# LasseWolter/laughter-detection-icsi

Measured on AMD Instinct MI355X. Metric: 1 s@16 kHz segments/sec (featurize+ResNet fwd/bwd), higher is better.
Workload: dtype f32 (64->64 and 32->32 convolutions: f16x2 split operands with per-tile power-of-two scales, f32 accumulate; error vs float64 within 1.5x of the exact-f32 kernels'); 1 GPU; BASELINE configs[2]: end-to-end featurize (HIP fbank 44 mel) + ResNetBigger resnet_base fwd/bwd + clip + Adam, random labels, dropout 0.5; global_batch=512, parallelism=dp1, overlap_wgrad=False, overlap_wgrad_small=True, bf16x3_convs=True, f16x2_convs=True, relu_bits=True, virtual_a1=True

## Files before the change

laughter-detection-icsi_amd/csrc/conv_h2.hip:

```cpp
#include "lad_common.h"
#include "lad_device.h"
#include "lad_b3_tile.h"
#include "lad_bn_math.h"
#include "lad_h2.h"

#include <algorithm>
#include <cstdlib>

namespace {
using namespace lad;
using namespace lad::b3t;

constexpr int KC = 32;
constexpr int ROWB = 128;
constexpr int FPIECES = KC * 4 / 16;

template <int C>
struct H2 {
    static constexpr int NSTAGE = C / KC;
    static constexpr int NCT = C / 16;
    static constexpr int PLANE_B = NCT * 1024;
    static constexpr int TAP_BYTES = 2 * PLANE_B;
    static constexpr int IMG_BYTES = TAPS * NSTAGE * TAP_BYTES;
    static constexpr int TAIL_BYTES = 16;
};

struct PackRec {
    const float *w;
    unsigned char *wt;
    int mode;
    int channels;
};
constexpr int PACK_SPLIT = 16;
template <int C>
__device__ __forceinline__ void pack_h2_image(const PackRec &rec, int part) {
    using K = H2<C>;
    __shared__ float smax[K::NSTAGE][16];
    __shared__ int kexp[K::NSTAGE];
    const int tid = threadIdx.x, lane = tid & 63, wave = tid >> 6;
    float m[K::NSTAGE];
#pragma unroll
    for (int s = 0; s < K::NSTAGE; ++s) m[s] = 0.f;
    static_assert((C * TAPS) % 4 == 0, "float4 groups stay inside one (co, ci range)");
    for (int idx4 = tid; idx4 < C * C * TAPS / 4; idx4 += 1024) {
        const float4 v = reinterpret_cast<const float4 *>(rec.w)[idx4];
        const float a[4] = {fabsf(v.x), fabsf(v.y), fabsf(v.z), fabsf(v.w)};
#pragma unroll
        for (int j = 0; j < 4; ++j) {
            const int idx = idx4 * 4 + j;
            const int co = idx / (C * TAPS), ci = (idx / TAPS) % C;
            const int k = rec.mode == 0 ? ci : co;
#pragma unroll
            for (int s = 0; s < K::NSTAGE; ++s) m[s] = (k / KC == s) ? fmaxf(m[s], a[j]) : m[s];
        }
    }
#pragma unroll
    for (int s = 0; s < K::NSTAGE; ++s) {
        const float v = wave_max64_dpp(m[s]);
        if (lane == 0) smax[s][wave] = v;
    }
    __syncthreads();
    if (tid < K::NSTAGE) {
        float v = 0.f;
        for (int w = 0; w < 16; ++w) v = fmaxf(v, smax[tid][w]);
        kexp[tid] = scale_exp(v);
        if (part == 0) reinterpret_cast<int *>(rec.wt + K::IMG_BYTES)[tid] = kexp[tid];
    }
    __syncthreads();
    unsigned short *out = reinterpret_cast<unsigned short *>(rec.wt);
    constexpr int SHARE = K::IMG_BYTES / 2 / PACK_SPLIT;
    for (int idx = part * SHARE + tid; idx < (part + 1) * SHARE; idx += 1024) {
        int t = idx;
        const int e = t & 7; t >>= 3;
        const int n = t & 15; t >>= 4;
        const int kq = t & 3; t >>= 2;
        const int ct = t % K::NCT; t /= K::NCT;
        const int plane = t & 1; t >>= 1;
        const int stage = t % K::NSTAGE;
        const int tap = t / K::NSTAGE;
        const int k = stage * KC + kq * 8 + e;
        const int nn = ct * 16 + n;
        const int co = rec.mode == 0 ? nn : k, ci = rec.mode == 0 ? k : nn;
        const int src_tap = rec.mode == 0 ? tap : TAPS - 1 - tap;
        const float v = rec.w[((int64_t)co * C + ci) * TAPS + src_tap] * pow2f(kexp[stage]);
        const _Float16 h1 = (_Float16)v;
        const _Float16 h2 = (_Float16)(v - (float)h1);
        out[idx] = __builtin_bit_cast(unsigned short, plane == 0 ? h1 : h2);
    }
}
template <int C>
__global__ __launch_bounds__(1024) void pack_h2_kernel(const PackRec *__restrict__ recs) {
    const PackRec rec = recs[blockIdx.x / PACK_SPLIT];
    const int part = blockIdx.x % PACK_SPLIT;
    if (C == 64 || (C == 0 && rec.channels == 64)) pack_h2_image<64>(rec, part);
    else pack_h2_image<32>(rec, part);
}

#ifdef LAD_STAMP
__device__ unsigned long long lad_dbg_h2[16 * 16384];
#define LAD_H2_STAMP(k) \
    if (threadIdx.x == 0 && blockIdx.x < 16384) lad_dbg_h2[blockIdx.x * 16 + (k)] = __builtin_amdgcn_s_memtime();
#else
#define LAD_H2_STAMP(k)
#endif

constexpr int NSLOT = 3;
constexpr int H2_EPI_ANY = -1;
constexpr int h2_epi(bool bias, int addend, bool partials, bool from_bits) {
    return (bias ? 1 : 0) | (addend << 1) | (partials ? 8 : 0) | (from_bits ? 16 : 0);
}
template <int C, int RB, bool STAT, bool INBN, int EPI>
__global__ __launch_bounds__(THREADS, RB == 1 ? 3 : 2) void conv_h2_kernel(const float *__restrict__ in, const unsigned char *__restrict__ wt,
                                                             const float *__restrict__ bias, const float *addend,
                                                             const unsigned long long *__restrict__ abits, float *out,
                                                             float *__restrict__ partials, Geom g, B3Stat bst,
                                                             const float *__restrict__ in_coef) {
    using K = H2<C>;
    constexpr int NSTAGE = K::NSTAGE, NCT = K::NCT, PLANE_B = K::PLANE_B, TAP_BYTES = K::TAP_BYTES;
    constexpr int TMW = TM * RB, NRT = 2 * RB;
    constexpr int NPRE = ((TMW + 2 * 47) * FPIECES + THREADS - 1) / THREADS;
    constexpr int CPS = TAPS;
    constexpr int KP = (CPS - NSLOT) < CPS / 2 ? (CPS - NSLOT) : CPS / 2;
    static_assert(CPS % NSLOT == 0 && NPRE <= 32, "every stage starts in ring slot 0; staging geometry");
    extern __shared__ __attribute__((aligned(128))) unsigned char smem_b[];
    const int tid = threadIdx.x, lane = tid & 63, wave = __builtin_amdgcn_readfirstlane(tid >> 6);
    const int halo = g.Wp + 1;
    const int nrows = TMW + 2 * halo;
    const int main_bytes = max(NSLOT * TAP_BYTES + nrows * ROWB, TM * (C + 4) * 4);
    unsigned char *b_s = smem_b;
    unsigned char *a_s = b_s + NSLOT * TAP_BYTES;
    unsigned char *mask_s = smem_b + main_bytes;
    float *smax = reinterpret_cast<float *>(mask_s + TMW);
    const unsigned per_x = (gridDim.x + 7u) / 8u;
    const unsigned tile_id = (blockIdx.x % 8u) * per_x + blockIdx.x / 8u;
    const int64_t q0 = (int64_t)tile_id * TMW;
    if (q0 >= g.rows) return;

    LAD_H2_STAMP(0)
    constexpr int NW_TAP = TAP_BYTES / (THREADS * 16);
    static_assert(TAP_BYTES % (THREADS * 16) == 0 && NW_TAP >= 1, "the DMA count per tap must not depend on the wave");
    auto issue_tap = [&](int tap, int stage, int slot) {
        const unsigned char *src = wt + (int64_t)(tap * NSTAGE + stage) * TAP_BYTES;
        unsigned char *dst = b_s + slot * TAP_BYTES;
#pragma unroll
        for (int r = 0; r < NW_TAP; ++r)
            dma16(src + (r * THREADS + tid) * 16, lds_addr(dst + (r * THREADS + wave * 64) * 16));
    };
    const int *wexp = reinterpret_cast<const int *>(wt + K::IMG_BYTES);

    const int64_t start = q0 - halo;
    const int64_t first = start < 0 ? 0 : start;
    const int row_lo = (int)(first - start);
    const int64_t span_rows = min(g.rows - first, (int64_t)(nrows - row_lo));
    auto voff = [&](int u) {
        const int idx = u * THREADS + tid;
        return idx < nrows * FPIECES ? ((idx >> 3) - row_lo) * (C * 4) + (idx & 7) * 16 : -1;
    };
    auto stage_rsrc = [&](int stage) {
        return make_rsrc(reinterpret_cast<const unsigned char *>(in) + first * (C * 4) + stage * (KC * 4), span_rows * (C * 4) - stage * (KC * 4));
    };
    unsigned keep_bits = 0;
    u32x4 pre[NPRE];
    auto activate = [&](int stage) {
        float m = 0.f;
        f32x4 sc = {0.f, 0.f, 0.f, 0.f}, sh = sc;
        if (INBN) {
            sc = *reinterpret_cast<const f32x4 *>(in_coef + stage * KC + (tid & 7) * 4);
            sh = *reinterpret_cast<const f32x4 *>(in_coef + C + stage * KC + (tid & 7) * 4);
        }
#pragma unroll
        for (int u = 0; u < NPRE; ++u) {
            if (INBN) pre[u] = bn_relu_piece(pre[u], sc, sh, (keep_bits >> u) & 1u);
            const float4 f = as_f4(pre[u]);
            m = fmaxf(fmaxf(m, fmaxf(fabsf(f.x), fabsf(f.y))), fmaxf(fabsf(f.z), fabsf(f.w)));
        }
        m = wave_max64_dpp(m);
        if (lane == 0) smax[wave] = m;
    };
    auto tile_exp = [&]() { return scale_exp(fmaxf(fmaxf(smax[0], smax[1]), fmaxf(smax[2], smax[3]))); };
    auto put_all = [&](float scl) {
#pragma unroll
        for (int u = 0; u < NPRE; ++u) {
            const int idx = u * THREADS + tid;
            if (idx < nrows * FPIECES) {
                const int row = idx >> 3, piece = idx & 7;
                const float4 f = as_f4(pre[u]);
                unsigned a1, a2, b1, b2;
                split2_pair(f.x * scl, f.y * scl, a1, a2);
                split2_pair(f.z * scl, f.w * scl, b1, b2);
                const unsigned off = (unsigned)row * ROWB + ((((piece >> 1) ^ (row & 6)) << 4) | ((piece & 1) << 3));
                *reinterpret_cast<u32x2 *>(a_s + off) = u32x2{a1, b1};
                *reinterpret_cast<u32x2 *>(a_s + (off ^ 64u)) = u32x2{a2, b2};
            }
        }
    };

    {
        const __amdgpu_buffer_rsrc_t in_r = stage_rsrc(0);
#pragma unroll
        for (int u = 0; u < NPRE; ++u) pre[u] = buf_load16(in_r, voff(u));
    }
#pragma unroll
    for (int k = 0; k < NSLOT - 1; ++k) issue_tap(k, 0, k);
    for (int j = tid; j < TMW; j += THREADS) mask_s[j] = interior_row32((uint32_t)q0 + (uint32_t)j, g) ? 1 : 0;
    if (INBN) {
#pragma unroll
        for (int u = 0; u < NPRE; ++u)
            keep_bits |= (interior_row32((uint32_t)(start + ((u * THREADS + tid) >> 3)), g) ? 1u : 0u) << u;
    }
    LAD_H2_STAMP(1)
    activate(0);
    __syncthreads();
    int ktot = tile_exp() + wexp[0];
    put_all(pow2f(ktot - wexp[0]));
    LAD_H2_STAMP(2)

    const int m = lane & 15, kq = lane >> 4;
    const int rl = wave * 32 + m + halo - 1;
    const unsigned char *b_lane = b_s + kq * 256 + m * 16;

    f32x4 acc[NRT][NCT];
#pragma unroll
    for (int r = 0; r < NRT; ++r)
#pragma unroll
        for (int c = 0; c < NCT; ++c) acc[r][c] = f32x4{0.f, 0.f, 0.f, 0.f};

#pragma unroll
    for (int stage = 0; stage < NSTAGE; ++stage) {
        const bool last = stage + 1 == NSTAGE;
#pragma unroll
        for (int tap = 0; tap < TAPS; ++tap) {
            const int kc = tap;
            const int slot = kc % NSLOT;
            {
                constexpr int YOUNGER = NSLOT - 2;
                if (!last) {
                    if (kc > KP && kc <= KP + NSLOT - 1) wait_dma_fixed<YOUNGER, NPRE, NW_TAP>();
                    else wait_dma_fixed<YOUNGER, 0, NW_TAP>();
                } else {
                    if (CPS - 1 - kc >= YOUNGER) wait_dma_fixed<YOUNGER, 0, NW_TAP>();
                    else wait_dma_fixed<0, 0, NW_TAP>();
                }
                __syncthreads();
                const int kn = kc + NSLOT - 1;
                if (kn < CPS) issue_tap(kn, stage, kn % NSLOT);
                else if (!last) issue_tap(kn - CPS, stage + 1, kn % NSLOT);
                if (kc == KP && !last) {
                    const __amdgpu_buffer_rsrc_t in_r = stage_rsrc(stage + 1);
#pragma unroll
                    for (int u = 0; u < NPRE; ++u) pre[u] = buf_load16(in_r, voff(u));
                }
            }
            const int rt = rl + (tap / 3 - 1) * g.Wp + (tap % 3);
            const unsigned a1o = (unsigned)rt * ROWB + ((unsigned)(kq ^ (rt & 6)) << 4);
            const unsigned a2o = a1o ^ 64u;
            const int boff = slot * TAP_BYTES;
            f16x8 a1[NRT], a2[NRT];
#pragma unroll
            for (int r = 0; r < NRT; ++r) {
                const int roff = ((r >> 1) * TM + (r & 1) * 16) * ROWB;
                a1[r] = *reinterpret_cast<const f16x8 *>(a_s + a1o + roff);
                a2[r] = *reinterpret_cast<const f16x8 *>(a_s + a2o + roff);
            }
#pragma unroll
            for (int c = 0; c < NCT; ++c) {
                const f16x8 b1 = *reinterpret_cast<const f16x8 *>(b_lane + boff + c * 1024);
                const f16x8 b2 = *reinterpret_cast<const f16x8 *>(b_lane + boff + PLANE_B + c * 1024);
#pragma unroll
                for (int r = 0; r < NRT; ++r) acc[r][c] = __builtin_amdgcn_mfma_f32_16x16x32_f16(a1[r], b2, acc[r][c], 0, 0, 0);
#pragma unroll
                for (int r = 0; r < NRT; ++r) acc[r][c] = __builtin_amdgcn_mfma_f32_16x16x32_f16(a2[r], b1, acc[r][c], 0, 0, 0);
#pragma unroll
                for (int r = 0; r < NRT; ++r) acc[r][c] = __builtin_amdgcn_mfma_f32_16x16x32_f16(a1[r], b1, acc[r][c], 0, 0, 0);
            }
        }
#ifdef LAD_STAMP
        if (threadIdx.x == 0 && blockIdx.x < 16384) lad_dbg_h2[blockIdx.x * 16 + 3 + 2 * stage] = __builtin_amdgcn_s_memtime();
#endif
        if (!last) {
            activate(stage + 1);
            __syncthreads();
            const int kw = wexp[stage + 1];
            const int kn = min(tile_exp() + kw, ktot + 8);
            const int d = kn - ktot;
            if (d != 0) {
#pragma unroll
                for (int r = 0; r < NRT; ++r)
#pragma unroll
                    for (int c = 0; c < NCT; ++c)
#pragma unroll
                        for (int j = 0; j < 4; ++j) acc[r][c][j] = __builtin_ldexpf(acc[r][c][j], d);
            }
            ktot = kn;
            const int ka = kn - kw;
            put_all(ka >= -126 ? pow2f(ka) : 0.f);
        }
#ifdef LAD_STAMP
        if (threadIdx.x == 0 && blockIdx.x < 16384) lad_dbg_h2[blockIdx.x * 16 + 4 + 2 * stage] = __builtin_amdgcn_s_memtime();
#endif
    }
    __syncthreads();
    LAD_H2_STAMP(11)
#pragma unroll
    for (int rb = 0; rb < RB; ++rb) {
        const int64_t qs = q0 + rb * TM;
        if (rb > 0) {
            if (qs >= g.rows) break;
            __syncthreads();
        }
        auto store_acc = [&](float *my) {
#pragma unroll
            for (int rr = 0; rr < 2; ++rr)
#pragma unroll
                for (int c = 0; c < NCT; ++c)
#pragma unroll
                    for (int j = 0; j < 4; ++j)
                        my[(rr * 16 + (lane >> 4) * 4 + j) * (C + 4) + c * 16 + m] = __builtin_ldexpf(acc[rb * 2 + rr][c][j], -ktot);
        };
        if constexpr (EPI == H2_EPI_ANY)
            b3_epilogue<C, STAT>(store_acc, bias, addend, abits, out, partials, mask_s + rb * TM, reinterpret_cast<float *>(smem_b), qs, g.rows, bst);
        else
            h2_epilogue<C, STAT, (EPI & 1) != 0, (EPI >> 1) & 3, (EPI & 8) != 0, (EPI & 16) != 0>(
                store_acc, bias, addend, abits, out, partials, mask_s + rb * TM, reinterpret_cast<float *>(smem_b), qs, g.rows, bst);
    }
    LAD_H2_STAMP(12)
}

template <int C, int RB>
size_t h2_lds_bytes(const Geom &g) {
    using K = H2<C>;
    const int nrows = TM * RB + 2 * (g.Wp + 1);
    const size_t main_bytes = std::max<size_t>(NSLOT * K::TAP_BYTES + (size_t)nrows * ROWB, (size_t)TM * (C + 4) * 4);
    return main_bytes + TM * RB + 16;
}

int h2_two_rounds() {
    static int n = 0;
    if (n == 0) {
        int dev = 0;
        hipDeviceProp_t prop;
        n = (hipGetDevice(&dev) == hipSuccess && hipGetDeviceProperties(&prop, dev) == hipSuccess && prop.multiProcessorCount > 0)
                ? 4 * prop.multiProcessorCount : 1024;
    }
    return n;
}

struct H2Args {
    const float *in, *in_coef;
    const unsigned char *wt;
    const float *bias, *addend;
    const unsigned long long *abits;
    float *out, *partials;
    B3Stat bst;
    Geom g;
    hipStream_t stream;
};

template <int C, int RB, bool STAT, bool INBN, int EPI>
int launch_h2_form(const H2Args &a) {
    static lad::DeviceOnce attr_set;
    if (!attr_set) {
        LAD_HIP_CHECK(hipFuncSetAttribute((const void *)conv_h2_kernel<C, RB, STAT, INBN, EPI>, hipFuncAttributeMaxDynamicSharedMemorySize, 96 * 1024));
        attr_set = true;
    }
    const int64_t tiles = ceil_div(a.g.rows, TM * RB);
    hipLaunchKernelGGL((conv_h2_kernel<C, RB, STAT, INBN, EPI>), dim3((unsigned)(ceil_div(tiles, 8) * 8)), dim3(THREADS), (h2_lds_bytes<C, RB>(a.g)),
                       a.stream, a.in, a.wt, a.bias, a.addend, a.abits, a.out, a.partials, a.g, a.bst, a.in_coef);
    return check_launch("conv_h2_kernel");
}

template <int C, int RB, bool STAT, bool INBN>
int launch_h2_rb(const H2Args &a) {
    const int form = h2_epi(a.bias != nullptr, a.addend == nullptr ? H2_ADD_NONE : a.abits == nullptr ? H2_ADD_PLAIN : H2_ADD_GATED,
                            a.partials != nullptr, STAT && a.bst.bits != nullptr);
#define LAD_H2_FORM(...)                                                                                                           \
    if (form == h2_epi(__VA_ARGS__)) return launch_h2_form<C, RB, STAT, INBN, h2_epi(__VA_ARGS__)>(a);
    if constexpr (STAT) {
        LAD_H2_FORM(false, H2_ADD_NONE, true, false)
        LAD_H2_FORM(false, H2_ADD_GATED, true, true)
    } else {
        LAD_H2_FORM(true, H2_ADD_NONE, true, false)
        LAD_H2_FORM(true, H2_ADD_PLAIN, true, false)
        if constexpr (!INBN) {
            LAD_H2_FORM(false, H2_ADD_NONE, false, false)
            LAD_H2_FORM(false, H2_ADD_PLAIN, false, false)
            LAD_H2_FORM(false, H2_ADD_GATED, false, false)
        }
    }
#undef LAD_H2_FORM
    return launch_h2_form<C, RB, STAT, INBN, H2_EPI_ANY>(a);
}

template <int C, bool STAT, bool INBN>
int launch_h2(const float *in, const float *in_coef, const void *wt, const float *bias, const float *addend, const uint64_t *abits,
              float *out, float *partials, const B3Stat &bst, int64_t batch, int32_t H, int32_t W, void *stream, const char *who) {
    const Geom g = make_geom(batch, H, W);
    LAD_REQUIRE(g.rows < ((int64_t)1 << 31) && g.img < (1 << 20), "%s: more than 2^31 rows, or an image of more than 2^20 positions", who);
    LAD_REQUIRE(W <= 46, "%s: image too wide for the tile (W = %d)", who, W);
    const H2Args a{in, in_coef, (const unsigned char *)wt, bias, addend, (const unsigned long long *)abits, out, partials, bst, g, (hipStream_t)stream};
    if (ceil_div(g.rows, TM * 2) < h2_two_rounds()) return launch_h2_rb<C, 1, STAT, INBN>(a);
    return launch_h2_rb<C, 2, STAT, INBN>(a);
}
}

extern "C" int64_t lad_conv_h2_packed_weight_bytes(int32_t channels) {
    if (channels == 64) return H2<64>::IMG_BYTES + H2<64>::TAIL_BYTES;
    if (channels == 32) return H2<32>::IMG_BYTES + H2<32>::TAIL_BYTES;
    return -1;
}

extern "C" int lad_conv_h2_pack_weights_multi(const void *table, int32_t n, int32_t channels, void *stream) {
    using namespace lad;
    LAD_REQUIRE(table && n >= 1, "lad_conv_h2_pack_weights_multi: empty table");
    static_assert(sizeof(PackRec) == 24, "record layout");
    if (channels == 64) hipLaunchKernelGGL(pack_h2_kernel<64>, dim3(n * PACK_SPLIT), dim3(1024), 0, (hipStream_t)stream, (const PackRec *)table);
    else if (channels == 32) hipLaunchKernelGGL(pack_h2_kernel<32>, dim3(n * PACK_SPLIT), dim3(1024), 0, (hipStream_t)stream, (const PackRec *)table);
    else if (channels == 0) hipLaunchKernelGGL(pack_h2_kernel<0>, dim3(n * PACK_SPLIT), dim3(1024), 0, (hipStream_t)stream, (const PackRec *)table);
    else return fail(LAD_ERR_INVALID, "lad_conv_h2_pack_weights_multi: 64 or 32 channels, or 0 = per record (got %d)", channels);
    return check_launch("pack_h2_kernel");
}

extern "C" int lad_conv_h2(const float *in, const float *in_coef, const void *wt, const float *bias, const float *addend,
                           const uint64_t *addend_bits, float *out, float *partials, const float *bn_x, const uint64_t *bn_bits,
                           const float *bn_coef, int64_t batch, int32_t H, int32_t W, int32_t channels, void *stream) {
    using namespace lad;
    const char *who = "lad_conv_h2";
    LAD_REQUIRE(batch >= 1 && H >= 1 && W >= 1, "%s: bad geometry", who);
    LAD_REQUIRE(in && wt && out, "%s: null buffer", who);
    LAD_REQUIRE(addend_bits == nullptr || addend != nullptr, "%s: sign bits without an addend", who);
    LAD_REQUIRE((const void *)in != (const void *)out, "%s: the convolution cannot run in place", who);
    const bool stat = bn_x != nullptr;
    LAD_REQUIRE(!stat || (partials && bn_coef), "%s: the BatchNorm sums need partials and bn_coef", who);
    LAD_REQUIRE(stat || bn_bits == nullptr, "%s: bn_bits without bn_x", who);
    LAD_REQUIRE(!(stat && in_coef), "%s: an input BatchNorm and the backward sums are not combined", who);
    LAD_REQUIRE(channels == 64 || (addend_bits == nullptr && bn_bits == nullptr), "%s: sign bits are kept for 64-channel activations only", who);
    const B3Stat bst{bn_x, (const unsigned long long *)bn_bits, bn_coef};
    if (channels == 64) {
        if (stat) return launch_h2<64, true, false>(in, nullptr, wt, bias, addend, addend_bits, out, partials, bst, batch, H, W, stream, who);
        if (in_coef) return launch_h2<64, false, true>(in, in_coef, wt, bias, addend, addend_bits, out, partials, bst, batch, H, W, stream, who);
        return launch_h2<64, false, false>(in, nullptr, wt, bias, addend, addend_bits, out, partials, bst, batch, H, W, stream, who);
    }
    if (channels == 32) {
        if (stat) return launch_h2<32, true, false>(in, nullptr, wt, bias, addend, addend_bits, out, partials, bst, batch, H, W, stream, who);
        if (in_coef) return launch_h2<32, false, true>(in, in_coef, wt, bias, addend, addend_bits, out, partials, bst, batch, H, W, stream, who);
        return launch_h2<32, false, false>(in, nullptr, wt, bias, addend, addend_bits, out, partials, bst, batch, H, W, stream, who);
    }
    return fail(LAD_ERR_INVALID, "%s: 64 or 32 channels (got %d)", who, channels);
}

#ifdef LAD_STAMP
extern "C" int lad_debug_read_h2_stamps(unsigned long long *host_dst, int64_t n) {
    return hipMemcpyFromSymbol(host_dst, HIP_SYMBOL(lad_dbg_h2), n * sizeof(unsigned long long)) == hipSuccess ? 0 : -2;
}
#endif
```

laughter-detection-icsi_amd/csrc/lad_b3_tile.h:

```cpp
#pragma once
#include "lad_common.h"
#include "lad_device.h"

namespace lad {
namespace b3t {

constexpr int TAPS = 9;
constexpr int TM = 128;
constexpr int THREADS = 256;

struct B3Stat {
    const float *x;
    const unsigned long long *bits;
    const float *coef;
};

struct B3Scatter {
    const int *rowoff;
    int64_t base_row;
    int64_t span_rows;
    int64_t part_tile;
};

template <int C, bool STAT, bool SCATTER = false, class StoreAcc, class MaskT>
__device__ __forceinline__ void b3_epilogue(StoreAcc store_acc, const float *__restrict__ bias, const float *addend,
                                            const unsigned long long *__restrict__ abits, float *out, float *__restrict__ partials,
                                            const MaskT *mask_tile, float *out_s, int64_t q0, int64_t rows, const B3Stat &bst,
                                            const B3Scatter &sct = B3Scatter{nullptr, 0, 0, 0}) {
    constexpr int LDO = C + 4, LPR = C / 4, RPI = 64 / LPR, ITER = 32 / RPI, STEP = RPI * C * 4;
    const int tid = (int)threadIdx.x, lane = tid & 63, wave = tid >> 6;
    float *my = out_s + wave * 32 * LDO;
    store_acc(my);
    const int c4 = lane % LPR, rsub = lane / LPR;
    const int64_t row0 = SCATTER ? sct.base_row : q0;
    const int64_t tile_rows = SCATTER ? sct.span_rows : rows - q0;
    const int64_t tile_bytes = tile_rows * (C * 4);
    const int voff = ((wave * 32 + rsub) * C + c4 * 4) * 4;
    const int woff = (wave * 32 + rsub) * 8;
    int ro[SCATTER ? ITER : 1];
    if (SCATTER) {
#pragma unroll
        for (int it = 0; it < ITER; ++it) ro[it] = sct.rowoff[wave * 32 + it * RPI + rsub];
    }
    auto off16 = [&](int it) { return SCATTER ? (ro[SCATTER ? it : 0] < 0 ? -1 : ro[SCATTER ? it : 0] * (C * 4) + c4 * 16) : voff + it * STEP; };
    auto off8 = [&](int it) { return SCATTER ? (ro[SCATTER ? it : 0] < 0 ? -1 : ro[SCATTER ? it : 0] * 8) : woff + it * RPI * 8; };
    const __amdgpu_buffer_rsrc_t out_r = make_rsrc(out + row0 * C, tile_bytes);
    f32x4 bv = {0.f, 0.f, 0.f, 0.f};
    if (bias != nullptr) bv = *reinterpret_cast<const f32x4 *>(bias + c4 * 4);
    f32x4 s1 = {0.f, 0.f, 0.f, 0.f}, s2 = s1;
    f32x4 fsc = s1, fsh = s1, mu = s1, is = s1, mul = s1, isl = s1;
    if (STAT) {
        fsc = *reinterpret_cast<const f32x4 *>(bst.coef + 0 * C + c4 * 4);
        fsh = *reinterpret_cast<const f32x4 *>(bst.coef + 1 * C + c4 * 4);
        mu = *reinterpret_cast<const f32x4 *>(bst.coef + 2 * C + c4 * 4);
        is = *reinterpret_cast<const f32x4 *>(bst.coef + 3 * C + c4 * 4);
        mul = *reinterpret_cast<const f32x4 *>(bst.coef + 4 * C + c4 * 4);
        isl = *reinterpret_cast<const f32x4 *>(bst.coef + 5 * C + c4 * 4);
    }
    const bool from_bits = STAT && bst.bits != nullptr;
    auto gate = [&](u32x4 v, u32x2 w) {
        const unsigned lo = w.x >> c4, hi = w.y >> c4;
        v.x = (lo & 1u) ? v.x : 0u;
        v.y = (lo & 0x10000u) ? v.y : 0u;
        v.z = (hi & 1u) ? v.z : 0u;
        v.w = (hi & 0x10000u) ? v.w : 0u;
        return v;
    };
    constexpr int NI = STAT ? ITER / 2 : ITER;
#pragma unroll
    for (int i0 = 0; i0 < ITER; i0 += NI) {
        u32x4 adv[NI], bx[STAT ? NI : 1];
        u32x2 wv[NI], bw[STAT ? NI : 1];
        if (addend != nullptr) {
            const __amdgpu_buffer_rsrc_t add_r = make_rsrc(addend + row0 * C, tile_bytes);
#pragma unroll
            for (int u = 0; u < NI; ++u) adv[u] = buf_load16(add_r, off16(i0 + u));
            if (abits != nullptr) {
                const __amdgpu_buffer_rsrc_t bits_r = make_rsrc(abits + row0, tile_rows * 8);
#pragma unroll
                for (int u = 0; u < NI; ++u) wv[u] = buf_load8(bits_r, off8(i0 + u));
            }
        }
        if (STAT) {
            const __amdgpu_buffer_rsrc_t x_r = make_rsrc(bst.x + row0 * C, tile_bytes);
#pragma unroll
            for (int u = 0; u < NI; ++u) bx[u] = buf_load16(x_r, off16(i0 + u));
            if (from_bits) {
                const __amdgpu_buffer_rsrc_t w_r = make_rsrc(bst.bits + row0, tile_rows * 8);
#pragma unroll
                for (int u = 0; u < NI; ++u) bw[u] = buf_load8(w_r, off8(i0 + u));
            }
        }
#pragma unroll
        for (int u = 0; u < NI; ++u) {
            const int it = i0 + u;
            const int row = it * RPI + rsub;
            const float keep = SCATTER ? (ro[SCATTER ? it : 0] < 0 ? 0.f : 1.f) : (float)mask_tile[wave * 32 + row];
            f32x4 t = *reinterpret_cast<const f32x4 *>(my + row * LDO + c4 * 4);
            t += bv;
            if (addend != nullptr) t += __builtin_bit_cast(f32x4, abits != nullptr ? gate(adv[u], wv[u]) : adv[u]);
            t *= keep;
            buf_store16(__builtin_bit_cast(u32x4, t), out_r, off16(it));
            if (!STAT) {
                s1 += t;
                s2 = __builtin_elementwise_fma(t, t, s2);
            } else {
                const f32x4 xv = __builtin_bit_cast(f32x4, bx[u]);
                f32x4 d;
                if (from_bits) {
                    d = __builtin_bit_cast(f32x4, gate(__builtin_bit_cast(u32x4, t), bw[u]));
                } else {
                    const f32x4 yv = __builtin_elementwise_fma(xv, fsc, fsh);
                    d.x = yv.x > 0.f ? t.x : 0.f;
                    d.y = yv.y > 0.f ? t.y : 0.f;
                    d.z = yv.z > 0.f ? t.z : 0.f;
                    d.w = yv.w > 0.f ? t.w : 0.f;
                }
                const f32x4 tx = (xv - mu) - mul;
                const f32x4 xh = __builtin_elementwise_fma(tx, is, tx * isl);
                s1 += d;
                s2 = __builtin_elementwise_fma(d, xh, s2);
            }
        }
    }
    if (partials == nullptr) return;
    *reinterpret_cast<f32x4 *>(my + (rsub * 2 + 0) * C + c4 * 4) = s1;
    *reinterpret_cast<f32x4 *>(my + (rsub * 2 + 1) * C + c4 * 4) = s2;
    __syncthreads();
    if (tid < 2 * C) {
        const int k = tid / C, co = tid - k * C;
        float s = 0.0f;
#pragma unroll
        for (int w = 0; w < 4; ++w)
#pragma unroll
            for (int rs = 0; rs < RPI; ++rs) s += out_s[w * 32 * LDO + (rs * 2 + k) * C + co];
        partials[((SCATTER ? sct.part_tile : q0 / TM) * 2 + k) * C + co] = s;
    }
}

enum : int { H2_ADD_NONE = 0, H2_ADD_PLAIN = 1, H2_ADD_GATED = 2 };
template <int C, bool STAT, bool HAS_BIAS, int ADDEND, bool HAS_PARTIALS, bool FROM_BITS, class StoreAcc>
__device__ __forceinline__ void h2_epilogue(StoreAcc store_acc, const float *__restrict__ bias, const float *addend,
                                            const unsigned long long *__restrict__ abits, float *out, float *__restrict__ partials,
                                            const unsigned char *mask_tile, float *out_s, int64_t q0, int64_t rows, const B3Stat &bst) {
    static_assert(!FROM_BITS || STAT, "sign bits of the consuming BatchNorm: STAT launches only");
    static_assert(!STAT || HAS_PARTIALS, "the BatchNorm sums need partials");
    constexpr int LDO = C + 4, LPR = C / 4, RPI = 64 / LPR, ITER = 32 / RPI, STEP = RPI * C * 4;
    const int tid = (int)threadIdx.x, lane = tid & 63, wave = tid >> 6;
    float *my = out_s + wave * 32 * LDO;
    store_acc(my);
    const int c4 = lane % LPR, rsub = lane / LPR;
    const int64_t tile_rows = rows - q0;
    const int64_t tile_bytes = tile_rows * (C * 4);
    const int voff = ((wave * 32 + rsub) * C + c4 * 4) * 4;
    const int woff = (wave * 32 + rsub) * 8;
    const __amdgpu_buffer_rsrc_t out_r = make_rsrc(out + q0 * C, tile_bytes);
    f32x4 bv = {0.f, 0.f, 0.f, 0.f};
    if constexpr (HAS_BIAS) bv = *reinterpret_cast<const f32x4 *>(bias + c4 * 4);
    f32x4 s1 = {0.f, 0.f, 0.f, 0.f}, s2 = s1;
    f32x4 fsc = s1, fsh = s1, mu = s1, is = s1, mul = s1, isl = s1;
    if constexpr (STAT) {
        if constexpr (!FROM_BITS) {
            fsc = *reinterpret_cast<const f32x4 *>(bst.coef + 0 * C + c4 * 4);
            fsh = *reinterpret_cast<const f32x4 *>(bst.coef + 1 * C + c4 * 4);
        }
        mu = *reinterpret_cast<const f32x4 *>(bst.coef + 2 * C + c4 * 4);
        is = *reinterpret_cast<const f32x4 *>(bst.coef + 3 * C + c4 * 4);
        mul = *reinterpret_cast<const f32x4 *>(bst.coef + 4 * C + c4 * 4);
        isl = *reinterpret_cast<const f32x4 *>(bst.coef + 5 * C + c4 * 4);
    }
    auto gate = [&](u32x4 v, u32x2 w) {
        const unsigned lo = w.x >> c4, hi = w.y >> c4;
        v.x = (lo & 1u) ? v.x : 0u;
        v.y = (lo & 0x10000u) ? v.y : 0u;
        v.z = (hi & 1u) ? v.z : 0u;
        v.w = (hi & 0x10000u) ? v.w : 0u;
        return v;
    };
    constexpr int NI = (STAT || ADDEND == H2_ADD_GATED) ? ITER / 2 : ITER;
#pragma unroll
    for (int i0 = 0; i0 < ITER; i0 += NI) {
        u32x4 adv[ADDEND != H2_ADD_NONE ? NI : 1], bx[STAT ? NI : 1];
        u32x2 wv[ADDEND == H2_ADD_GATED ? NI : 1], bw[FROM_BITS ? NI : 1];
        if constexpr (ADDEND != H2_ADD_NONE) {
            const __amdgpu_buffer_rsrc_t add_r = make_rsrc(addend + q0 * C, tile_bytes);
#pragma unroll
            for (int u = 0; u < NI; ++u) adv[u] = buf_load16(add_r, voff + (i0 + u) * STEP);
            if constexpr (ADDEND == H2_ADD_GATED) {
                const __amdgpu_buffer_rsrc_t bits_r = make_rsrc(abits + q0, tile_rows * 8);
#pragma unroll
                for (int u = 0; u < NI; ++u) wv[u] = buf_load8(bits_r, woff + (i0 + u) * RPI * 8);
            }
        }
        if constexpr (STAT) {
            const __amdgpu_buffer_rsrc_t x_r = make_rsrc(bst.x + q0 * C, tile_bytes);
#pragma unroll
            for (int u = 0; u < NI; ++u) bx[u] = buf_load16(x_r, voff + (i0 + u) * STEP);
            if constexpr (FROM_BITS) {
                const __amdgpu_buffer_rsrc_t w_r = make_rsrc(bst.bits + q0, tile_rows * 8);
#pragma unroll
                for (int u = 0; u < NI; ++u) bw[u] = buf_load8(w_r, woff + (i0 + u) * RPI * 8);
            }
        }
#pragma unroll
        for (int u = 0; u < NI; ++u) {
            const int it = i0 + u;
            const int row = it * RPI + rsub;
            const float keep = (float)mask_tile[wave * 32 + row];
            f32x4 t = *reinterpret_cast<const f32x4 *>(my + row * LDO + c4 * 4);
            t += bv;
            if constexpr (ADDEND == H2_ADD_GATED) t += __builtin_bit_cast(f32x4, gate(adv[u], wv[u]));
            else if constexpr (ADDEND == H2_ADD_PLAIN) t += __builtin_bit_cast(f32x4, adv[u]);
            t *= keep;
            buf_store16(__builtin_bit_cast(u32x4, t), out_r, voff + it * STEP);
            if constexpr (!STAT) {
                if constexpr (HAS_PARTIALS) {
                    s1 += t;
                    s2 = __builtin_elementwise_fma(t, t, s2);
                }
            } else {
                const f32x4 xv = __builtin_bit_cast(f32x4, bx[u]);
                f32x4 d;
                if constexpr (FROM_BITS) {
                    d = __builtin_bit_cast(f32x4, gate(__builtin_bit_cast(u32x4, t), bw[u]));
                } else {
                    const f32x4 yv = __builtin_elementwise_fma(xv, fsc, fsh);
                    d.x = yv.x > 0.f ? t.x : 0.f;
                    d.y = yv.y > 0.f ? t.y : 0.f;
                    d.z = yv.z > 0.f ? t.z : 0.f;
                    d.w = yv.w > 0.f ? t.w : 0.f;
                }
                const f32x4 tx = (xv - mu) - mul;
                const f32x4 xh = __builtin_elementwise_fma(tx, is, tx * isl);
                s1 += d;
                s2 = __builtin_elementwise_fma(d, xh, s2);
            }
        }
    }
    if constexpr (HAS_PARTIALS) {
        *reinterpret_cast<f32x4 *>(my + (rsub * 2 + 0) * C + c4 * 4) = s1;
        *reinterpret_cast<f32x4 *>(my + (rsub * 2 + 1) * C + c4 * 4) = s2;
        __syncthreads();
        if (tid < 2 * C) {
            const int k = tid / C, co = tid - k * C;
            float s = 0.0f;
#pragma unroll
            for (int w = 0; w < 4; ++w)
#pragma unroll
                for (int rs = 0; rs < RPI; ++rs) s += out_s[w * 32 * LDO + (rs * 2 + k) * C + co];
            partials[(q0 / TM * 2 + k) * C + co] = s;
        }
    }
}

template <int TAP_BYTES>
__device__ __forceinline__ int dma_per_tap(int wave) {
    int n = 0;
#pragma unroll
    for (int r = 0; r * THREADS * 16 < TAP_BYTES; ++r) n += ((r * THREADS + wave * 64) * 16 < TAP_BYTES) ? 1 : 0;
    return n;
}

template <int TAPS_YOUNGER, int EXTRA>
__device__ __forceinline__ void wait_dma(int nw_tap) {
    static_assert(2 * TAPS_YOUNGER + EXTRA <= 63, "vmcnt is a 6-bit field");
    if (nw_tap == 2) asm volatile("s_waitcnt vmcnt(%0)" ::"n"(2 * TAPS_YOUNGER + EXTRA) : "memory");
    else if (nw_tap == 1) asm volatile("s_waitcnt vmcnt(%0)" ::"n"(TAPS_YOUNGER + EXTRA) : "memory");
    else asm volatile("s_waitcnt vmcnt(%0)" ::"n"(EXTRA) : "memory");
}
template <int TAPS_YOUNGER, int EXTRA, int NW_TAP>
__device__ __forceinline__ void wait_dma_fixed() {
    static_assert(NW_TAP * TAPS_YOUNGER + EXTRA <= 63, "vmcnt is a 6-bit field");
    asm volatile("s_waitcnt vmcnt(%0)" ::"n"(NW_TAP * TAPS_YOUNGER + EXTRA) : "memory");
}

}
}
```

Baseline: 50110 segments/s.

## Prefetch epilogue addend/stat loads during last conv stage and pipeline sub-tiles

For RB==2 launches whose epilogue reads global data (addend, gate bits, BN input), the coefficient and first sub-tile loads are now issued during the last stage's final taps. This hides their latency behind the remaining MFMA work. The epilogue is restructured so each sub-tile issues the next sub-tile's loads (or the next row block's) before consuming the current ones, which double-buffers global reads. It also sets NI per config, and a sched_barrier fence is used for the widest case. In exchange it holds more registers live across the main loop, which risks spills or lower occupancy, and it adjusts the waitcnt accounting accordingly.

```diff
diff --git a/laughter-detection-icsi_amd/csrc/conv_h2.hip b/laughter-detection-icsi_amd/csrc/conv_h2.hip
--- a/laughter-detection-icsi_amd/csrc/conv_h2.hip
+++ b/laughter-detection-icsi_amd/csrc/conv_h2.hip
@@ -109,6 +109,18 @@
 constexpr int h2_epi(bool bias, int addend, bool partials, bool from_bits) {
     return (bias ? 1 : 0) | (addend << 1) | (partials ? 8 : 0) | (from_bits ? 16 : 0);
 }
+template <int C, int RB, bool STAT, int EPI>
+struct H2EpiPlan {
+    static constexpr int ADDEND = EPI == H2_EPI_ANY ? H2_ADD_NONE : (EPI >> 1) & 3;
+    static constexpr bool FROM_BITS = EPI != H2_EPI_ANY && (EPI & 16) != 0;
+    static constexpr bool READS = EPI != H2_EPI_ANY && (STAT || ADDEND != H2_ADD_NONE);
+    static constexpr bool AHEAD = READS && RB == 2;
+    static constexpr int ITER = 32 / (64 / (C / 4));
+    static constexpr bool WIDEST = FROM_BITS && ADDEND == H2_ADD_GATED;
+    static constexpr int NI = (STAT || ADDEND == H2_ADD_GATED) && (RB == 1 || WIDEST) ? ITER / 2 : ITER;
+    static constexpr int TAP = TAPS - NSLOT;
+    static constexpr bool FENCE = AHEAD && WIDEST;
+};
 template <int C, int RB, bool STAT, bool INBN, int EPI>
 __global__ __launch_bounds__(THREADS, RB == 1 ? 3 : 2) void conv_h2_kernel(const float *__restrict__ in, const unsigned char *__restrict__ wt,
                                                              const float *__restrict__ bias, const float *addend,
@@ -225,6 +237,13 @@
 #pragma unroll
         for (int c = 0; c < NCT; ++c) acc[r][c] = f32x4{0.f, 0.f, 0.f, 0.f};
 
+    using EP = H2EpiPlan<C, RB, STAT, EPI>;
+    using Req = H2Req<C, STAT && EPI != H2_EPI_ANY, EP::ADDEND, EP::FROM_BITS, EP::NI>;
+    static_assert(EP::TAP >= CPS - NSLOT && EP::TAP < CPS, "requests go behind the last weight DMA of the last stage");
+    using Coef = H2Coef<C, STAT && EPI != H2_EPI_ANY, EPI != H2_EPI_ANY && (EPI & 1) != 0, EP::FROM_BITS>;
+    Req req[RB + 1];
+    Coef coef;
+
 #pragma unroll
     for (int stage = 0; stage < NSTAGE; ++stage) {
         const bool last = stage + 1 == NSTAGE;
@@ -238,8 +257,14 @@
                     if (kc > KP && kc <= KP + NSLOT - 1) wait_dma_fixed<YOUNGER, NPRE, NW_TAP>();
                     else wait_dma_fixed<YOUNGER, 0, NW_TAP>();
                 } else {
-                    if (CPS - 1 - kc >= YOUNGER) wait_dma_fixed<YOUNGER, 0, NW_TAP>();
-                    else wait_dma_fixed<0, 0, NW_TAP>();
+                    constexpr int RQ = EP::AHEAD ? Coef::LOADS + Req::LOADS : 0;
+                    if (CPS - 1 - kc >= YOUNGER) {
+                        if (kc > EP::TAP) wait_dma_fixed<YOUNGER, RQ, NW_TAP>();
+                        else wait_dma_fixed<YOUNGER, 0, NW_TAP>();
+                    } else {
+                        if (kc > EP::TAP) wait_dma_fixed<0, RQ, NW_TAP>();
+                        else wait_dma_fixed<0, 0, NW_TAP>();
+                    }
                 }
                 __syncthreads();
                 const int kn = kc + NSLOT - 1;
@@ -249,6 +274,12 @@
                     const __amdgpu_buffer_rsrc_t in_r = stage_rsrc(stage + 1);
 #pragma unroll
                     for (int u = 0; u < NPRE; ++u) pre[u] = buf_load16(in_r, voff(u));
+                }
+                if constexpr (EP::AHEAD) {
+                    if (last && kc == EP::TAP) {
+                        h2_coefs(coef, bias, bst);
+                        h2_request(req[0], 0, addend, abits, q0, g.rows, bst);
+                    }
                 }
             }
             const int rt = rl + (tap / 3 - 1) * g.Wp + (tap % 3);
@@ -299,6 +330,7 @@
         if (threadIdx.x == 0 && blockIdx.x < 16384) lad_dbg_h2[blockIdx.x * 16 + 4 + 2 * stage] = __builtin_amdgcn_s_memtime();
 #endif
     }
+    if constexpr (EP::FENCE) __builtin_amdgcn_sched_barrier(0);
     __syncthreads();
     LAD_H2_STAMP(11)
 #pragma unroll
@@ -319,9 +351,25 @@
         };
         if constexpr (EPI == H2_EPI_ANY)
             b3_epilogue<C, STAT>(store_acc, bias, addend, abits, out, partials, mask_s + rb * TM, reinterpret_cast<float *>(smem_b), qs, g.rows, bst);
-        else
-            h2_epilogue<C, STAT, (EPI & 1) != 0, (EPI >> 1) & 3, (EPI & 8) != 0, (EPI & 16) != 0>(
-                store_acc, bias, addend, abits, out, partials, mask_s + rb * TM, reinterpret_cast<float *>(smem_b), qs, g.rows, bst);
+        else {
+            auto coefs = [&]() {
+                if constexpr (EP::AHEAD) {
+                    return coef;
+                } else {
+                    Coef c;
+                    h2_coefs(c, bias, bst);
+                    return c;
+                }
+            };
+            auto request_next = [&]() {
+                if constexpr (EP::AHEAD) {
+                    if (rb + 1 < RB && qs + TM < g.rows) h2_request(req[rb + 1], 0, addend, abits, qs + TM, g.rows, bst);
+                }
+            };
+            h2_epilogue<C, STAT, (EPI & 1) != 0, EP::ADDEND, (EPI & 8) != 0, EP::FROM_BITS, EP::NI, EP::AHEAD>(
+                store_acc, coefs, addend, abits, out, partials, mask_s + rb * TM, reinterpret_cast<float *>(smem_b), qs, g.rows, bst,
+                req[rb], request_next);
+        }
     }
     LAD_H2_STAMP(12)
 }
diff --git a/laughter-detection-icsi_amd/csrc/lad_b3_tile.h b/laughter-detection-icsi_amd/csrc/lad_b3_tile.h
--- a/laughter-detection-icsi_amd/csrc/lad_b3_tile.h
+++ b/laughter-detection-icsi_amd/csrc/lad_b3_tile.h
@@ -139,11 +139,74 @@
 }
 
 enum : int { H2_ADD_NONE = 0, H2_ADD_PLAIN = 1, H2_ADD_GATED = 2 };
-template <int C, bool STAT, bool HAS_BIAS, int ADDEND, bool HAS_PARTIALS, bool FROM_BITS, class StoreAcc>
-__device__ __forceinline__ void h2_epilogue(StoreAcc store_acc, const float *__restrict__ bias, const float *addend,
+template <int C, bool STAT, int ADDEND, bool FROM_BITS, int NI>
+struct H2Req {
+    static constexpr int ITER = 32 / (64 / (C / 4));
+    static_assert(NI >= 1 && ITER % NI == 0, "a sub-tile is a whole number of records");
+    static_assert(!FROM_BITS || STAT, "sign bits of the consuming BatchNorm: STAT launches only");
+    static constexpr int LOADS = NI * ((ADDEND != H2_ADD_NONE ? 1 : 0) + (ADDEND == H2_ADD_GATED ? 1 : 0) + (STAT ? 1 : 0) + (FROM_BITS ? 1 : 0));
+    u32x4 adv[ADDEND != H2_ADD_NONE ? NI : 1], bx[STAT ? NI : 1];
+    u32x2 wv[ADDEND == H2_ADD_GATED ? NI : 1], bw[FROM_BITS ? NI : 1];
+};
+template <int C, bool STAT, bool HAS_BIAS, bool FROM_BITS>
+struct H2Coef {
+    static constexpr int LOADS = (HAS_BIAS ? 1 : 0) + (STAT ? (FROM_BITS ? 4 : 6) : 0);
+    f32x4 bv, fsc, fsh, mu, is, mul, isl;
+};
+template <int C, bool STAT, bool HAS_BIAS, bool FROM_BITS>
+__device__ __forceinline__ void h2_coefs(H2Coef<C, STAT, HAS_BIAS, FROM_BITS> &co, const float *__restrict__ bias, const B3Stat &bst) {
+    const int c4 = ((int)threadIdx.x & 63) % (C / 4);
+    co.bv = f32x4{0.f, 0.f, 0.f, 0.f};
+    co.fsc = co.fsh = co.mu = co.is = co.mul = co.isl = co.bv;
+    if constexpr (HAS_BIAS) co.bv = *reinterpret_cast<const f32x4 *>(bias + c4 * 4);
+    if constexpr (STAT) {
+        if constexpr (!FROM_BITS) {
+            co.fsc = *reinterpret_cast<const f32x4 *>(bst.coef + 0 * C + c4 * 4);
+            co.fsh = *reinterpret_cast<const f32x4 *>(bst.coef + 1 * C + c4 * 4);
+        }
+        co.mu = *reinterpret_cast<const f32x4 *>(bst.coef + 2 * C + c4 * 4);
+        co.is = *reinterpret_cast<const f32x4 *>(bst.coef + 3 * C + c4 * 4);
+        co.mul = *reinterpret_cast<const f32x4 *>(bst.coef + 4 * C + c4 * 4);
+        co.isl = *reinterpret_cast<const f32x4 *>(bst.coef + 5 * C + c4 * 4);
+    }
+}
+template <int C, bool STAT, int ADDEND, bool FROM_BITS, int NI>
+__device__ __forceinline__ void h2_request(H2Req<C, STAT, ADDEND, FROM_BITS, NI> &rq, int i0, const float *addend,
+                                           const unsigned long long *__restrict__ abits, int64_t q0, int64_t rows, const B3Stat &bst) {
+    constexpr int LPR = C / 4, RPI = 64 / LPR, STEP = RPI * C * 4;
+    const int tid = (int)threadIdx.x, lane = tid & 63, wave = tid >> 6;
+    const int c4 = lane % LPR, rsub = lane / LPR;
+    const int64_t tile_rows = rows - q0;
+    const int64_t tile_bytes = tile_rows * (C * 4);
+    const int voff = ((wave * 32 + rsub) * C + c4 * 4) * 4;
+    const int woff = (wave * 32 + rsub) * 8;
+    if constexpr (ADDEND != H2_ADD_NONE) {
+        const __amdgpu_buffer_rsrc_t add_r = make_rsrc(addend + q0 * C, tile_bytes);
+#pragma unroll
+        for (int u = 0; u < NI; ++u) rq.adv[u] = buf_load16(add_r, voff + (i0 + u) * STEP);
+        if constexpr (ADDEND == H2_ADD_GATED) {
+            const __amdgpu_buffer_rsrc_t bits_r = make_rsrc(abits + q0, tile_rows * 8);
+#pragma unroll
+            for (int u = 0; u < NI; ++u) rq.wv[u] = buf_load8(bits_r, woff + (i0 + u) * RPI * 8);
+        }
+    }
+    if constexpr (STAT) {
+        const __amdgpu_buffer_rsrc_t x_r = make_rsrc(bst.x + q0 * C, tile_bytes);
+#pragma unroll
+        for (int u = 0; u < NI; ++u) rq.bx[u] = buf_load16(x_r, voff + (i0 + u) * STEP);
+        if constexpr (FROM_BITS) {
+            const __amdgpu_buffer_rsrc_t w_r = make_rsrc(bst.bits + q0, tile_rows * 8);
+#pragma unroll
+            for (int u = 0; u < NI; ++u) rq.bw[u] = buf_load8(w_r, woff + (i0 + u) * RPI * 8);
+        }
+    }
+}
+
+template <int C, bool STAT, bool HAS_BIAS, int ADDEND, bool HAS_PARTIALS, bool FROM_BITS, int NI, bool AHEAD, class StoreAcc, class Coefs, class Next>
+__device__ __forceinline__ void h2_epilogue(StoreAcc store_acc, Coefs coefs, const float *addend,
                                             const unsigned long long *__restrict__ abits, float *out, float *__restrict__ partials,
-                                            const unsigned char *mask_tile, float *out_s, int64_t q0, int64_t rows, const B3Stat &bst) {
-    static_assert(!FROM_BITS || STAT, "sign bits of the consuming BatchNorm: STAT launches only");
+                                            const unsigned char *mask_tile, float *out_s, int64_t q0, int64_t rows, const B3Stat &bst,
+                                            const H2Req<C, STAT, ADDEND, FROM_BITS, NI> &first, Next request_next) {
     static_assert(!STAT || HAS_PARTIALS, "the BatchNorm sums need partials");
     constexpr int LDO = C + 4, LPR = C / 4, RPI = 64 / LPR, ITER = 32 / RPI, STEP = RPI * C * 4;
     const int tid = (int)threadIdx.x, lane = tid & 63, wave = tid >> 6;
@@ -153,22 +216,10 @@
     const int64_t tile_rows = rows - q0;
     const int64_t tile_bytes = tile_rows * (C * 4);
     const int voff = ((wave * 32 + rsub) * C + c4 * 4) * 4;
-    const int woff = (wave * 32 + rsub) * 8;
     const __amdgpu_buffer_rsrc_t out_r = make_rsrc(out + q0 * C, tile_bytes);
-    f32x4 bv = {0.f, 0.f, 0.f, 0.f};
-    if constexpr (HAS_BIAS) bv = *reinterpret_cast<const f32x4 *>(bias + c4 * 4);
+    const H2Coef<C, STAT, HAS_BIAS, FROM_BITS> co = coefs();
+    const f32x4 bv = co.bv, fsc = co.fsc, fsh = co.fsh, mu = co.mu, is = co.is, mul = co.mul, isl = co.isl;
     f32x4 s1 = {0.f, 0.f, 0.f, 0.f}, s2 = s1;
-    f32x4 fsc = s1, fsh = s1, mu = s1, is = s1, mul = s1, isl = s1;
-    if constexpr (STAT) {
-        if constexpr (!FROM_BITS) {
-            fsc = *reinterpret_cast<const f32x4 *>(bst.coef + 0 * C + c4 * 4);
-            fsh = *reinterpret_cast<const f32x4 *>(bst.coef + 1 * C + c4 * 4);
-        }
-        mu = *reinterpret_cast<const f32x4 *>(bst.coef + 2 * C + c4 * 4);
-        is = *reinterpret_cast<const f32x4 *>(bst.coef + 3 * C + c4 * 4);
-        mul = *reinterpret_cast<const f32x4 *>(bst.coef + 4 * C + c4 * 4);
-        isl = *reinterpret_cast<const f32x4 *>(bst.coef + 5 * C + c4 * 4);
-    }
     auto gate = [&](u32x4 v, u32x2 w) {
         const unsigned lo = w.x >> c4, hi = w.y >> c4;
         v.x = (lo & 1u) ? v.x : 0u;
@@ -177,31 +228,17 @@
         v.w = (hi & 0x10000u) ? v.w : 0u;
         return v;
     };
-    constexpr int NI = (STAT || ADDEND == H2_ADD_GATED) ? ITER / 2 : ITER;
-#pragma unroll
-    for (int i0 = 0; i0 < ITER; i0 += NI) {
-        u32x4 adv[ADDEND != H2_ADD_NONE ? NI : 1], bx[STAT ? NI : 1];
-        u32x2 wv[ADDEND == H2_ADD_GATED ? NI : 1], bw[FROM_BITS ? NI : 1];
-        if constexpr (ADDEND != H2_ADD_NONE) {
-            const __amdgpu_buffer_rsrc_t add_r = make_rsrc(addend + q0 * C, tile_bytes);
-#pragma unroll
-            for (int u = 0; u < NI; ++u) adv[u] = buf_load16(add_r, voff + (i0 + u) * STEP);
-            if constexpr (ADDEND == H2_ADD_GATED) {
-                const __amdgpu_buffer_rsrc_t bits_r = make_rsrc(abits + q0, tile_rows * 8);
-#pragma unroll
-                for (int u = 0; u < NI; ++u) wv[u] = buf_load8(bits_r, woff + (i0 + u) * RPI * 8);
-            }
-        }
-        if constexpr (STAT) {
-            const __amdgpu_buffer_rsrc_t x_r = make_rsrc(bst.x + q0 * C, tile_bytes);
-#pragma unroll
-            for (int u = 0; u < NI; ++u) bx[u] = buf_load16(x_r, voff + (i0 + u) * STEP);
-            if constexpr (FROM_BITS) {
-                const __amdgpu_buffer_rsrc_t w_r = make_rsrc(bst.bits + q0, tile_rows * 8);
-#pragma unroll
-                for (int u = 0; u < NI; ++u) bw[u] = buf_load8(w_r, woff + (i0 + u) * RPI * 8);
-            }
-        }
+    constexpr int NREC = ITER / NI;
+    H2Req<C, STAT, ADDEND, FROM_BITS, NI> rq[NREC];
+    if constexpr (AHEAD) rq[0] = first;
+#pragma unroll
+    for (int k = 0; k < NREC; ++k) {
+        const int i0 = k * NI;
+        H2Req<C, STAT, ADDEND, FROM_BITS, NI> now;
+        if constexpr (!AHEAD) h2_request(now, i0, addend, abits, q0, rows, bst);
+        else if (k + 1 < NREC) h2_request(rq[k + 1 < NREC ? k + 1 : 0], i0 + NI, addend, abits, q0, rows, bst);
+        else request_next();
+        const H2Req<C, STAT, ADDEND, FROM_BITS, NI> &r = AHEAD ? rq[k] : now;
 #pragma unroll
         for (int u = 0; u < NI; ++u) {
             const int it = i0 + u;
@@ -209,8 +246,8 @@
             const float keep = (float)mask_tile[wave * 32 + row];
             f32x4 t = *reinterpret_cast<const f32x4 *>(my + row * LDO + c4 * 4);
             t += bv;
-            if constexpr (ADDEND == H2_ADD_GATED) t += __builtin_bit_cast(f32x4, gate(adv[u], wv[u]));
-            else if constexpr (ADDEND == H2_ADD_PLAIN) t += __builtin_bit_cast(f32x4, adv[u]);
+            if constexpr (ADDEND == H2_ADD_GATED) t += __builtin_bit_cast(f32x4, gate(r.adv[u], r.wv[u]));
+            else if constexpr (ADDEND == H2_ADD_PLAIN) t += __builtin_bit_cast(f32x4, r.adv[u]);
             t *= keep;
             buf_store16(__builtin_bit_cast(u32x4, t), out_r, voff + it * STEP);
             if constexpr (!STAT) {
@@ -219,10 +256,10 @@
                     s2 = __builtin_elementwise_fma(t, t, s2);
                 }
             } else {
-                const f32x4 xv = __builtin_bit_cast(f32x4, bx[u]);
+                const f32x4 xv = __builtin_bit_cast(f32x4, r.bx[u]);
                 f32x4 d;
                 if constexpr (FROM_BITS) {
-                    d = __builtin_bit_cast(f32x4, gate(__builtin_bit_cast(u32x4, t), bw[u]));
+                    d = __builtin_bit_cast(f32x4, gate(__builtin_bit_cast(u32x4, t), r.bw[u]));
                 } else {
                     const f32x4 yv = __builtin_elementwise_fma(xv, fsc, fsh);
                     d.x = yv.x > 0.f ? t.x : 0.f;
```

After: 50310 segments/s (median of 6 runs). Within noise of the previous version (+0.4%).
